# ShawnNew/Detectron2-CenterNet

Measured on AMD Instinct MI355X. Metric: images/sec at 512x512 (infer bs=64), higher is better.
Workload: dtype f16x3

## Files before the change

### detectron2-centernet_amd/csrc/api.hip

```cpp
#include "conv_common.h"
#include "../../include/ctdet_hip.h"
#include <stdarg.h>
#include <stdio.h>
#include <string.h>
#include <stdlib.h>
#include <atomic>

static thread_local char g_err[512] = "";
void ctdet_set_error(const char* fmt, ...) {
  va_list ap;
  va_start(ap, fmt);
  vsnprintf(g_err, sizeof(g_err), fmt, ap);
  va_end(ap);
}

thread_local int g_label_mode = 0;
static thread_local char g_label[128] = "";
bool ctdet_set_label(const char* fmt, ...) {
  va_list ap;
  va_start(ap, fmt);
  vsnprintf(g_label, sizeof(g_label), fmt, ap);
  va_end(ap);
  return g_label_mode == 2;
}
// ... 12 lines not shown
size_t dwconv3x3_wgrad_workspace_bytes(int, int, int, int, int);
int launch_dwconv3x3(const void*, int, const float*, void*, int, int, int, int, int, int, int, int, hipStream_t);
int launch_dwconv3x3_wgrad(const void*, int, const void*, int, float*, float*, float, int, int, int, int, int, int, hipStream_t);
size_t decode_workspace_bytes(int B, int H, int W, int C, int K);
int decode_status_words(int H, int W, int C, int K, long* ws_words, int* below_word);
int launch_decode(const DecArgs&, hipStream_t);
int launch_postprocess(const float*, const float*, const int*, int, int, int, float, const float*, float*, float*, int*,
                       int*, hipStream_t);
int launch_gaussian_radius(const int*, int, double*, int*, hipStream_t);
int launch_gaussian_targets(const float*, const int64_t*, const int*, int, int, int, int, int, float*, float*, float*,
                            int64_t*, uint8_t*, hipStream_t);
size_t focal_workspace_bytes(long numel);
int launch_focal_loss(const float*, const float*, const float*, int, int, int, int, float, void*, float*, float*, float*,
                      hipStream_t);
int launch_reg_l1(const float*, int, const uint8_t*, const int64_t*, const float*, int, int, int, float, float*, float*,
                  int, hipStream_t);
int launch_sgd(float*, const float*, float*, long, const float*, float, float, int, hipStream_t);
int launch_sgd_runs(float*, const float*, float*, long, const long*, const int*, const float*, const float*, int, float, int,
                    hipStream_t);

struct WgradArgs {
  const void* x; const void* dy; float* dw;
  int B, H, W, Cin, in_stride, Cout, Ho, Wo, dy_stride, R, S, stride, pad, dil, K, M, msplit;
  float scale;
  int lw, lh;
  int perm_rs, perm_cin, cin_real, cout_real;
};
int launch_grad_scatter_oihw(const void* const*, void* const*, const int*, const int*, const int*, const int*, int, hipStream_t);
int launch_pack_weights_batch(const void*, int, int, hipStream_t);
int launch_pack_weights_x3(const float*, void*, float*, int, int, int, int, int, int, int, int, int, int, hipStream_t);
int launch_pack_weights_x3_batch(const void*, int, int, hipStream_t);
int launch_split_weights(const float*, void*, long, hipStream_t);
bool dcn_offset_fused_ok(const ConvArgs& a);
int conv_pair_korder(const ConvArgs& a);
bool head_fused_x_ok(const HeadArgs& a, bool x3);
bool dcn_split_window_ok(const ConvArgs& a);
size_t chan_reduce_workspace_bytes(int C);
int launch_bn_train_fwd(const f16*, int, const f16*, int, f16*, int, int, int, const float*, const float*, float, float,
                        float*, float*, float*, float*, float*, float*, void*, int, hipStream_t);
int launch_bn_train_bwd(const f16*, int, const f16*, int, const f16*, int, const float*, const float*, const float*, int,
                        int, int, f16*, int, f16*, int, float*, float*, float, void*, hipStream_t);
int launch_conv_wgrad(const WgradArgs&, hipStream_t);
int launch_conv_wgrad_f32(const WgradArgs&, hipStream_t);
int launch_conv_wgrad_x3(const WgradArgs&, hipStream_t);
int launch_bn_train_fwd_f32(const float*, int, const float*, int, float*, int, int, int, const float*, const float*, float,
                            float, float*, float*, float*, float*, float*, float*, void*, int, hipStream_t);
int launch_bn_train_bwd_f32(const float*, int, const float*, int, const float*, int, const float*, const float*, const float*,
                            int, int, int, float*, int, float*, int, float*, float*, float, void*, hipStream_t);
int launch_bn_local_stats(const void*, int, int, int, int, int, double*, void*, int, hipStream_t);
int launch_bn_sync_fwd(const void*, int, const void*, int, void*, int, int, int, const double*, int, const float*, const float*,
                       float, float, float*, float*, float*, float*, float*, float*, int, int, hipStream_t);
int launch_bn_local_grad_sums(const void*, int, const void*, int, const void*, int, const float*, const float*, int, int, int, int,
                              int, double*, float*, float*, float, void*, int, hipStream_t);
int launch_bn_sync_bwd(const void*, int, const void*, int, const void*, int, const float*, const float*, const float*,
                       const double*, const double*, int, int, int, int, void*, int, void*, int, int, hipStream_t);
int launch_maxpool2x2_bwd_f32(const float*, int, const float*, int, float*, int, int, int, int, int, hipStream_t);
int launch_maxpool3x3s2_bwd(const void*, int, const void*, int, void*, int, int, int, int, int, int, int, int, int, hipStream_t);
int launch_ese_dot(const void*, int, const void*, int, int, int, int, int, float*, hipStream_t);
int launch_ese_bwd(const void*, int, const float*, const float*, void*, int, int, int, int, int, hipStream_t);
int launch_dwconvT_bwd_f32(const float*, int, const float*, int, const float*, float*, int, float*, int, int, int, int, int,
                           hipStream_t);
int launch_dcn_cols_f32(const float*, int, const float*, int, float*, int, int, int, int, int, hipStream_t);
int launch_dcn_col2im_coord_f32(const float*, const float*, int, const float*, int, float*, float*, int, int, int, int, int, int,
                                int, int, hipStream_t);
int launch_dcn_col2im_fused(const float*, int, int, const void*, const float*, const float*, int, const float*, int, float*, float*, int,
                            int, int, int, int, int, hipStream_t);
// ... 141 lines not shown
  }
  CTDET_CHECK(false, "dcnv2: bad compute dtype %d", d->compute_dtype);
}

int32_t ctdet_dcnv2_cols_supported(const ctdet_conv_desc* d, const void* x, const void* y) {
  ConvArgs a;
  if (fill_args(d, a) || d->compute_dtype != CTDET_DT_F16X3 || d->out_dtype != CTDET_DT_F32) return 0;
  a.x = x; a.y = const_cast<void*>(y);
  return dcn_split_window_ok(a) ? 1 : 0;
}

int32_t ctdet_dcnv2_fwd_cols(const ctdet_conv_desc* d, const void* x, const float* offset_mask, int32_t om_stride,
                             int32_t mask_is_prob, const void* w_packed, const float* scale, const float* bias, void* y,
                             float* cols_out, void* stream) {
  ConvArgs a;
  int rc = fill_args(d, a);
  if (rc) return rc;
  if (a.M == 0) return 0;
  CTDET_CHECK(x && w_packed && y && offset_mask && cols_out, "dcnv2_fwd_cols: null pointer");
  CTDET_CHECK(mask_is_prob >= CTDET_DCN_MASK_LOGIT && mask_is_prob <= CTDET_DCN_MASK_NONE, "dcnv2: mask mode %d", mask_is_prob);
  CTDET_CHECK(om_stride >= (mask_is_prob == CTDET_DCN_MASK_NONE ? 2 : 3) * d->R * d->S, "dcnv2: om_stride=%d < %d*R*S", om_stride,
              mask_is_prob == CTDET_DCN_MASK_NONE ? 2 : 3);
  CTDET_CHECK(d->compute_dtype == CTDET_DT_F16X3 && d->out_dtype == CTDET_DT_F32 && (((size_t)cols_out) & 15) == 0,
              "dcnv2_fwd_cols: the f16x3 mode's entry point (f32 tensors), 16-byte aligned columns");
  a.x = x; a.w = w_packed; a.scale = scale; a.bias = bias; a.res = nullptr; a.y = y;
  a.om = offset_mask; a.om_stride = om_stride; a.mask_is_prob = mask_is_prob;
  CTDET_CHECK(dcn_split_window_ok(a), "dcnv2_fwd_cols: shape not served by the LDS-window kernel (ask ctdet_dcnv2_cols_supported first)");
  a.cols_out = cols_out;
  return launch_conv_f32(a, true, true, (hipStream_t)stream);
}

int32_t ctdet_dcnv2_offset_supported(const ctdet_conv_desc* d) {
  ConvArgs a;
  if (fill_args(d, a) || d->compute_dtype != CTDET_DT_F16) return 0;
  a.y = nullptr;
  return dcn_offset_fused_ok(a) ? 1 : 0;
}

int32_t ctdet_dcnv2_offset_fwd(const ctdet_conv_desc* d, const void* x, const void* w_off_packed, const float* b_off,
                               float* om_out, int32_t om_out_stride, const void* w_packed, const float* scale,
                               const float* bias, void* y, void* stream) {
  ConvArgs a;
  int rc = fill_args(d, a);
  if (rc) return rc;
  if (a.M == 0) return 0;
  CTDET_CHECK(x && w_off_packed && b_off && w_packed && y, "dcnv2_offset: null pointer");
  CTDET_CHECK(d->compute_dtype == CTDET_DT_F16, "dcnv2_offset: f16 only");
  CTDET_CHECK(!om_out || (om_out_stride >= 28 && om_out_stride % 4 == 0 && ((size_t)om_out & 15) == 0),
              "dcnv2_offset: om_out needs a 16-byte aligned row of >= 28 floats (stride %d)", om_out_stride);
  a.x = x; a.w = w_packed; a.scale = scale; a.bias = bias; a.res = nullptr; a.y = y;
  a.w_off = w_off_packed; a.b_off = b_off; a.om_out = om_out; a.om_out_stride = om_out_stride;
  return launch_conv_f16(a, d->out_dtype, true, (hipStream_t)stream);
}

int32_t ctdet_preprocess(const void* img, int32_t img_dtype, void* out, int32_t out_dtype, int32_t B, int32_t H,
                         int32_t W, int32_t Hp, int32_t Wp, int64_t img_batch_stride, const float* mean3,
                         const float* std3, int32_t out_stride, int32_t border, void* stream) {
  CTDET_CHECK(img && out && mean3 && std3, "preprocess: null pointer");
  return launch_preprocess(img, img_dtype, out, out_dtype, B, H, W, Hp, Wp, (long)img_batch_stride, mean3, std3,
                           out_stride, border, (hipStream_t)stream);
}

static int head_args(const ctdet_head_desc* d, HeadArgs& a) {
  a.nheads = d->nheads; a.B = d->B; a.H = d->H; a.W = d->W; a.Cin = d->Cin; a.in_stride = d->in_stride;
  a.clamp_lo = d->clamp_lo; a.clamp_hi = d->clamp_hi;
  CTDET_CHECK(d->nheads >= 1 && d->nheads <= 4, "head_fused: nheads=%d out of range", d->nheads);
  for (int h = 0; h < d->nheads; ++h) {
    CTDET_CHECK(d->w2[h] && d->b2[h] && d->y[h], "head_fused: head %d: null pointer", h);
    a.w2[h] = d->w2[h]; a.b2[h] = (const float*)d->b2[h]; a.y[h] = (float*)d->y[h];
    a.y_stride[h] = d->y_stride[h]; a.cout[h] = d->cout[h]; a.act[h] = d->act[h];
  }
  return 0;
}

int32_t ctdet_head_fused_supported(int32_t compute_dtype, int32_t H, int32_t W, int32_t Cin, int32_t in_stride, const void* x) {
  HeadArgs a = {};
  a.x = x; a.H = H; a.W = W; a.Cin = Cin; a.in_stride = in_stride;
  if (compute_dtype != CTDET_DT_F16 && compute_dtype != CTDET_DT_F16X3) return 0;
  return head_fused_x_ok(a, compute_dtype == CTDET_DT_F16X3) ? 1 : 0;
}
// ... 457 lines not shown
```

### detectron2-centernet_amd/csrc/conv_f32.hip

```cpp
#include "conv_common.h"

template <int BP, int BC, int WP, int WC_, bool SP>
__global__ void __launch_bounds__(256) conv_f32_mfma_kernel(const ConvArgs a) {
  constexpr int KS = 16, EPV = 4;
  constexpr int TP = BP / WP / 16;
  constexpr int TC = BC / WC_ / 16;
  constexpr int A_LD = BP / 64;
  constexpr int BCL = BC < 64 ? 64 : BC;
  constexpr int B_LD = BCL / 64;
  constexpr int NLOAD = A_LD + B_LD;
  constexpr int STAGE = (BP + BCL) * 64;
  constexpr int NST = 3;
  static_assert(WP * WC_ == 4, "4 waves per workgroup");
  __shared__ __attribute__((aligned(16))) char smem[NST * STAGE];

  const int tid = threadIdx.x, lane = tid & 63;
  const int wave = __builtin_amdgcn_readfirstlane(tid >> 6);
  const int wp = wave / WC_, wc = wave % WC_;
  int m_tile, n_tile;
  if (!tile_of_block((a.M + BP - 1) / BP, a.Cout_pad / BC, m_tile, n_tile)) return;
  const int m0 = m_tile * BP, n0 = n_tile * BC;
  const float* __restrict__ x = (const float*)a.x;
  const float* __restrict__ w = (const float*)a.w;
  const float* zero = (const float*)g_zero_page;
// ... 626 lines not shown
    if (T == 8 && chunk + 1 < nch) {
      wait_vmcnt<0>();
      __builtin_amdgcn_s_barrier();
      asm volatile("" ::: "memory");
      sample(0, chunk + 1, pfn);
    }
#pragma unroll
    for (int p = 0; p < TP; ++p) pf[p] = pfn[p];
    if (TS < 2) {
#pragma unroll
      for (int c = 0; c < TC; ++c) wf[c] = wfn[c];
    }
  };
  for (int chunk = 0; chunk < nch; ++chunk) {
    const int s = chunk * 3;
    tap(s, chunk, std::integral_constant<int, 0>{});
    tap(s, chunk, std::integral_constant<int, 1>{});
    tap(s, chunk, std::integral_constant<int, 2>{});
    tap(s + 1, chunk, std::integral_constant<int, 3>{});
    tap(s + 1, chunk, std::integral_constant<int, 4>{});
    tap(s + 1, chunk, std::integral_constant<int, 5>{});
    tap(s + 2, chunk, std::integral_constant<int, 6>{});
    tap(s + 2, chunk, std::integral_constant<int, 7>{});
    tap(s + 2, chunk, std::integral_constant<int, 8>{});
  }

#pragma unroll
  for (int p = 0; p < TP; ++p) {
    const int m = (b * a.H + ty0 + prow) * a.W + tx0 + 8 * p + pcol;
    epilogue_tiles<float, TC>(a, m, n0, q, acc[p]);
  }
}

template <int TP, int BC, bool COLS = false, bool NM = false>
__global__ void __launch_bounds__(512 / TP, (TP == 1 && BC == 64) ? 4 : 2) dcn_split_window_kernel(const ConvArgs a) {
  constexpr int TH = 8, TW = 16, BP = 128, MG = 4;
  constexpr int NT = 512 / TP;
  static_assert(BC * 4 <= NT, "at most one weight piece per thread and tap (waves beyond BC / 16 fetch none)");
  constexpr int WR = TH + 2 + 2 * MG, WCOLS = TW + 2 + 2 * MG;
  constexpr int NPIECE = WR * WCOLS * 4;
  constexpr int W_LD = (NPIECE + NT - 1) / NT;
  constexpr int WINB = ((NPIECE + 63) / 64) * 1024;
  constexpr int GEOW = 9 * BP * 16, GEOC = 9 * BP * 4;
  constexpr int TC = BC / 16;
  constexpr int WST = BC * 64, NST = 2, STG = 3 * WST;
  static_assert(WINB + GEOW + GEOC + NST * STG <= ((TP == 2 || BC == 64) ? 81920 : 163840), "two workgroups / one (128 couts) per CU");
  __shared__ __attribute__((aligned(16))) char smem[WINB + GEOW + GEOC + NST * STG];
  char* const win = smem;
  char* const geow = smem + WINB;
  char* const geoc = smem + WINB + GEOW;
  char* const ring = smem + WINB + GEOW + GEOC;

  const int tid = threadIdx.x, lane = tid & 63;
  const int wave = __builtin_amdgcn_readfirstlane(tid >> 6);
  const int tiles_x = a.W / TW, tiles_y = a.H / TH;
  int m_tile, n_tile;
  if (!tile_of_block(a.B * tiles_y * tiles_x, a.Cout_pad / BC, m_tile, n_tile)) return;
  const int tx0 = (m_tile % tiles_x) * TW;
  const int ty0 = ((m_tile / tiles_x) % tiles_y) * TH;
  const int b = m_tile / (tiles_x * tiles_y);
  const int n0 = n_tile * BC;
  const float* zero = (const float*)g_zero_page;
  asm volatile("" : "+v"(zero));
  const float* ximg = (const float*)a.x + (long)b * a.H * a.W * a.in_stride;
  const int wy0 = ty0 - 1 - MG, wx0 = tx0 - 1 - MG;
  const int nch = a.Cin / 16;

  const int lrow = tid >> 2, slotw = tid & 3;
  const int gwk = slotw ^ swz(lrow);
  const float* wptr;
  {
    const int tt = lrow >> 4, r = lrow & 15;
    wptr = (const float*)a.w + (long)(n0 + cout_of<TC>(tt, r >> 2, r & 3)) * a.Kpad + gwk * 4;
  }
  auto issue_w = [&](int chunk, int tr, int st) {
    if (BC * 4 < NT && wave >= BC / 16) return;
#pragma unroll
    for (int ts = 0; ts < 3; ++ts)
      dma16(wptr + (tr * 3 + ts) * a.Cin + chunk * 16, ring + st * STG + ts * WST + wave * 1024);
  };
  int wofs[W_LD];
#pragma unroll
  for (int i = 0; i < W_LD; ++i) {
    const int pid = tid + NT * i;
    const int pw = pid >> 2, sl = pid & 3;
    const int wr = pw / WCOLS, wcn = pw - wr * WCOLS;
    const int y = wy0 + wr, x = wx0 + wcn;
    const bool ok = pid < NPIECE && y >= 0 && y < a.H && x >= 0 && x < a.W;
    wofs[i] = ok ? (y * a.W + x) * a.in_stride + (sl ^ (2 * (wr & 1))) * 4 : -1;
  }
  auto issue_window = [&](int chunk) {
#pragma unroll
    for (int i = 0; i < W_LD; ++i) {
      if (i < W_LD - 1 || (wave * 64 + NT * i) * 16 < WINB) {
        int o = wofs[i];
        asm volatile("" : "+v"(o));
        dma16(o >= 0 ? ximg + o + chunk * 16 : zero, win + (wave * 64 + NT * i) * 16);
      }
    }
  };
  issue_window(0);
  issue_w(0, 0, 0);

  {
    constexpr int GS = NT / 128;
    const int gp = tid & 127, gh = tid >> 7;
    const int py = ty0 + (gp >> 4), pxx = tx0 + (gp & 15);
    const float* omrow = a.om + ((long)(b * a.H + py) * a.W + pxx) * a.om_stride;
#pragma unroll
    for (int i = 0; i < (9 + GS - 1) / GS; ++i) {
      const int t = GS * i + gh;
      if (t < 9) {
        const int tr = t / 3, ts = t - 3 * tr;
        const float h_im = (float)(py - 1 + tr) + omrow[2 * t], w_im = (float)(pxx - 1 + ts) + omrow[2 * t + 1];
        const float mraw = NM ? 1.f : omrow[18 + t];
        const bool valid = h_im > -1.f && w_im > -1.f && h_im < (float)a.H && w_im < (float)a.W;
        const float mk = valid ? ((NM || a.mask_is_prob) ? mraw : ctdet_sigmoid_exact(mraw)) : 0.f;
        const float fh = floorf(h_im), fw = floorf(w_im);
        const int h_low = (int)fh, w_low = (int)fw;
        const float lh = valid ? h_im - fh : 0.f, lw = valid ? w_im - fw : 0.f, hh = 1.f - lh, hw = 1.f - lw;
        const int wr = h_low - wy0, wcn = w_low - wx0;
        const bool inside = wr >= 0 && wr + 1 < WR && wcn >= 0 && wcn + 1 < WCOLS;
        const bool oow = valid && !inside;
        const unsigned code = (valid && inside) ? ((unsigned)((wr * WCOLS + wcn) * 64) | ((unsigned)(wr & 1) << 5)) : (oow ? 0x80000000u : 0u);
        f32x4 gv;
        gv[0] = hh * hw * mk; gv[1] = hh * lw * mk; gv[2] = lh * hw * mk; gv[3] = lh * lw * mk;
        *(f32x4*)(geow + (t * BP + gp) * 16) = gv;
        *(unsigned*)(geoc + (t * BP + gp) * 4) = code;
      }
    }
  }
  wait_vmcnt<0>();
  __syncthreads();
  const int fr = lane & 15, q = lane >> 4;
  const int prow = TP == 2 ? 2 * wave + (fr >> 3) : wave, pcol = TP == 2 ? (fr & 7) : fr;
  const unsigned q4 = (unsigned)q << 4;

  struct Raw { f32x4 w[TP], v[TP][4]; };
  auto gather = [&](int t, int chunk, Raw& r) {
    unsigned code[TP];
    unsigned far = 0;
#pragma unroll
    for (int p = 0; p < TP; ++p) {
      const int px = prow * 16 + (TP == 2 ? 8 * p : 0) + pcol;
      r.w[p] = *(const f32x4*)(geow + (t * BP + px) * 16);
      code[p] = *(const unsigned*)(geoc + (t * BP + px) * 4);
      far |= code[p] >> 31;
    }
    const bool any_far = __builtin_amdgcn_ballot_w64(far != 0) != 0;
#pragma unroll
    for (int p = 0; p < TP; ++p) {
      const unsigned A = (code[p] & 0xFFFFu) ^ q4;
      const char* c0p = win + A;
      const char* c2p = win + (A ^ 32u) + WCOLS * 64;
      r.v[p][0] = *(const f32x4*)(c0p); r.v[p][1] = *(const f32x4*)(c0p + 64);
      r.v[p][2] = *(const f32x4*)(c2p); r.v[p][3] = *(const f32x4*)(c2p + 64);
      if (any_far) {
        const bool out = code[p] >> 31;
        const int py = ty0 + prow, pxx = tx0 + (TP == 2 ? 8 * p : 0) + pcol, tr = t / 3, ts = t - 3 * (t / 3);
        const float* omrow = a.om + ((long)(b * a.H + py) * a.W + pxx) * a.om_stride;
        float dh, dw;
        gload2_sync(omrow + 2 * t, dh, dw);
        const float h_im = (float)(py - 1 + tr) + dh, w_im = (float)(pxx - 1 + ts) + dw;
        const int h_low = (int)floorf(h_im), w_low = (int)floorf(w_im);
        const bool r0 = out && h_low >= 0, r1 = out && h_low + 1 <= a.H - 1, c0 = w_low >= 0, c1 = w_low + 1 <= a.W - 1;
        const long o0 = ((long)h_low * a.W + w_low) * a.in_stride, o2 = o0 + (long)a.W * a.in_stride;
        const float* base = ximg + chunk * 16 + q * 4;
        if (out) {
          gload4_sync_into((r0 && c0) ? base + o0 : zero, r.v[p][0]);
          gload4_sync_into((r0 && c1) ? base + o0 + a.in_stride : zero, r.v[p][1]);
          gload4_sync_into((r1 && c0) ? base + o2 : zero, r.v[p][2]);
          gload4_sync_into((r1 && c1) ? base + o2 + a.in_stride : zero, r.v[p][3]);
        }
      }
    }
  };
  float* const colp = (COLS && n0 == 0) ? a.cols_out + q * 4 : nullptr;
  auto blend = [&](const Raw& r, f16x8 (&b1)[TP], f16x8 (&b2)[TP], int t, int chunk) {
#pragma unroll
    for (int p = 0; p < TP; ++p) {
      f32x4 val;
#pragma unroll
      for (int e = 0; e < 4; ++e)
        val[e] = r.w[p][0] * r.v[p][0][e] + r.w[p][1] * r.v[p][1][e] + r.w[p][2] * r.v[p][2][e] + r.w[p][3] * r.v[p][3][e];
      if constexpr (COLS) {
        if (colp) {
          const long m = (long)(b * a.H + ty0 + prow) * a.W + tx0 + (TP == 2 ? 8 * p : 0) + pcol;
          *(f32x4*)(colp + m * (9L * a.Cin) + t * a.Cin + chunk * 16) = val;
        }
      }
      split_b(val, b1[p], b2[p]);
    }
  };

  f32x4 acc[TP][TC];
#pragma unroll
  for (int p = 0; p < TP; ++p)
// ... 399 lines not shown
    if (vec && !deform) {
      const int rc = launch_halo_split(a, s);
      if (rc <= 0) return rc;
    }
  }
  if (deform)
    return a.mask_is_prob == DCN_MASK_NONE ? launch_f32_deform<SP, true>(a, vec, bc, s) : launch_f32_deform<SP, false>(a, vec, bc, s);
  if (vec) {
    const bool big = ((long)a.M + 255) / 256 * (a.Cout_pad / bc) >= 512;
    const int kind = f32_uniform_k_ok(a) ? 1 : 0;
    switch (bc) {
      case 16: return launch_f32_mfma<256, 16, 4, 1, SP>(a, kind, s);
      case 32: return big ? launch_f32_mfma<256, 32, 4, 1, SP>(a, kind, s) : launch_f32_mfma<128, 32, 4, 1, SP>(a, kind, s);
      case 64: return big ? launch_f32_mfma<256, 64, 4, 1, SP>(a, kind, s) : launch_f32_mfma<128, 64, 2, 2, SP>(a, kind, s);
      case 128: return big ? launch_f32_mfma<256, 128, 2, 2, SP>(a, kind, s) : launch_f32_mfma<128, 128, 2, 2, SP>(a, kind, s);
    }
  }
  const int CP = (a.Cout + 3) & ~3;
  const long total = (long)a.M * CP;
  dim3 grid((unsigned)((total + 255) / 256));
  CTDET_KERNEL("conv_direct_%s_kernel<conv>", sp_name<SP>());
  hipLaunchKernelGGL((conv_direct_f32_kernel<false, SP>), grid, dim3(256), 0, s, a);
  CTDET_LAUNCH_CHECK();
  return 0;
}

bool dcn_split_window_ok(const ConvArgs& a) {
  const int bc = pick_bc(a.Cout);
  return f32_vector_ok(a, bc) && a.Cin % 16 == 0 && a.nsrc <= 1 && a.R == 3 && a.S == 3 && a.stride == 1 && a.pad == 1 && a.dil == 1 &&
         a.H % 8 == 0 && a.W % 16 == 0 && a.H <= 4094 && a.W <= 4094 && a.Kpad == a.K && a.Cout_pad % 64 == 0 && a.korder == 0 &&
         !(ctdet_tuning_flags() & (CTDET_TUNE_NO_F32_DCN_WINDOW | CTDET_TUNE_DCN_WINDOW_V1));
}

int launch_conv_f32(const ConvArgs& a, bool deform, bool split, hipStream_t s) {
  return split ? launch_conv_f32_t<true>(a, deform, s) : launch_conv_f32_t<false>(a, deform, s);
}

__global__ void __launch_bounds__(256) split_weights_kernel(const f32x4* __restrict__ src, f16x8* __restrict__ dst, long groups) {
  const long i = (long)blockIdx.x * 256 + threadIdx.x;
  if (i >= groups) return;
  const f32x4 w = src[i];
  f16x8 o;
#pragma unroll
  for (int j = 0; j < 4; ++j) {
    const f16 h = (f16)w[j];
    o[j] = h;
    o[4 + j] = (f16)(w[j] - (float)h);
  }
  dst[i] = o;
}

int launch_split_weights(const float* src, void* dst, long n, hipStream_t s) {
  CTDET_CHECK(n % 4 == 0 && (((size_t)src | (size_t)dst) & 15) == 0, "split_weights: needs 16-byte aligned buffers of a multiple of 4 floats");
  if (n == 0) return 0;
  const long groups = n / 4;
  hipLaunchKernelGGL(split_weights_kernel, dim3((unsigned)((groups + 255) / 256)), dim3(256), 0, s, (const f32x4*)src, (f16x8*)dst,
                     groups);
  CTDET_LAUNCH_CHECK();
  return 0;
}
```

### detectron2-centernet_amd/layers/deform_conv.py

```python
import math

import torch
from torch import nn
from torch.nn.modules.utils import _pair

from .. import ops
from ..ops import ACT_NONE, ACT_RELU, DCN_MASK_NONE, DCN_MASK_PROB, F16, F32
from . import hipnn


def _check_supported(groups, deformable_groups, stride, dilation):
    if groups != 1 or deformable_groups != 1:
        raise NotImplementedError("HIP DCNv2 supports groups=1, deformable_groups=1 (all CenterNet uses)")


def modulated_deform_conv(input, offset, mask, weight, bias=None, stride=1, padding=0, dilation=1, groups=1,
                          deformable_groups=1):
    if not input.is_cuda:
        raise NotImplementedError("Deformable Conv is not supported on CPUs!")
    _check_supported(groups, deformable_groups, stride, dilation)
    return _deform_conv_nchw(input, [offset, mask], weight, bias, stride, padding, dilation, DCN_MASK_PROB,
                             "modulated_deform_conv")


# ... 85 lines not shown
                                  self.groups, self.deformable_groups)
        if self.norm is not None:
            x = self.norm(x)
        if self.activation is not None:
            x = self.activation(x)
        return x


class DCN(nn.Module):

    def __init__(self, in_channels, out_channels, kernel_size, stride, padding, dilation=1, deformable_groups=1):
        super().__init__()
        _check_supported(1, deformable_groups, stride, dilation)
        self.in_channels, self.out_channels = in_channels, out_channels
        self.kernel_size = _pair(kernel_size)
        self.stride, self.padding, self.dilation = stride, padding, dilation
        self.deformable_groups = deformable_groups
        self.weight = nn.Parameter(torch.Tensor(out_channels, in_channels, *self.kernel_size))
        self.bias = nn.Parameter(torch.Tensor(out_channels))
        n = in_channels * self.kernel_size[0] * self.kernel_size[1]
        stdv = 1.0 / math.sqrt(n)
        self.weight.data.uniform_(-stdv, stdv)
        self.bias.data.zero_()
        kh, kw = self.kernel_size
        self.conv_offset_mask = nn.Conv2d(in_channels, deformable_groups * 3 * kh * kw, kernel_size=self.kernel_size,
                                          stride=stride, padding=padding, bias=True)
        self.conv_offset_mask.weight.data.zero_()
        self.conv_offset_mask.bias.data.zero_()

    def hip_forward(self, x, ctx, bn=None, act=ACT_NONE):
        p = hipnn.packed(self, "dcn", ctx.compute, self.weight, bn, self.bias, self.stride, self.padding, self.dilation,
                         cout_align=64 if ctx.compute == F16 else None)
        com = self.conv_offset_mask
        if ctx.compute == F16 and x.shape[3] % 32 == 0:
            p_off = hipnn.packed(com, "conv", ctx.compute, com.weight, None, com.bias, com.stride[0], com.padding[0], com.dilation[0])
            if ops.dcnv2_offset_supported(x, p_off, p):
                return ops.dcnv2_offset(x, p_off, p, act=act)
        om = hipnn.conv_module(x, com, None, ACT_NONE, ctx=ctx, out_dtype=torch.float32)
        return ops.dcnv2(x, om, p, act=act)

    def forward(self, x):
        ctx = hipnn.Ctx(F16 if x.dtype == torch.float16 else F32)
        xh = x.permute(0, 2, 3, 1).contiguous()
        if torch.is_grad_enabled() and (x.requires_grad or self.weight.requires_grad):
            from ..ops_train import ConvFn, DCNFn
            om = ConvFn.apply(xh, self.conv_offset_mask.weight, self.conv_offset_mask.bias, self.stride, self.padding,
                              False, True, 1.0)
            y = DCNFn.apply(xh, om, self.weight, self.bias, False, 1.0)
        else:
            y = self.hip_forward(xh, ctx)
        return hipnn.to_nchw_view(y, self.out_channels)


class DeformConvV2(nn.Module):

    def __init__(self, chi, cho):
        super().__init__()
        self.actf = nn.Sequential(nn.BatchNorm2d(cho, momentum=0.1), nn.ReLU(inplace=True))
        self.conv = DCN(chi, cho, kernel_size=(3, 3), stride=1, padding=1, dilation=1, deformable_groups=1)
        nn.init.uniform_(self.actf[0].weight.data)

    def hip_forward(self, x, ctx):
        return self.conv.hip_forward(x, ctx, bn=self.actf[0], act=ACT_RELU)

    def forward(self, x):
        ctx = hipnn.Ctx(F16 if x.dtype == torch.float16 else F32)
        return hipnn.to_nchw_view(self.hip_forward(hipnn.to_nhwc(x, ctx), ctx), self.conv.out_channels)
# ... 1 lines not shown
```

### detectron2-centernet_amd/ops.py

```python
import ctypes as C
import os
import math

import torch

from . import _lib
from ._lib import (ACT_NONE, ACT_RELU, ACT_SIGMOID_CLAMP, DCN_MASK_LOGIT, DCN_MASK_NONE, DCN_MASK_PROB, F16, F16X3, F32, U8,
                   ConvDesc, HeadDesc)

_TORCH_DT = {F16: torch.float16, F32: torch.float32}

PROFILE_ON = False
PROFILE = []
PROFILE_REP = 5


class _Prof:
    def __init__(self, p, M, deform, out_dt, nsrc=1, flops=None):
        self.on = PROFILE_ON
        if self.on:
            _lib.lib().ctdet_set_label_mode(1)
            self.flops = flops if flops is not None else 2.0 * M * p.Cout * p.R * p.S * p.Cin_real
            osz = 2 if out_dt == F16 else 4
            if p is not None:
# ... 494 lines not shown
    mask_is_prob = int(mask_is_prob)
    if mask_is_prob not in (DCN_MASK_LOGIT, DCN_MASK_PROB, DCN_MASK_NONE):
        raise ValueError(f"dcnv2: mask mode {mask_is_prob}")
    if p.compute == F16 and p.Cout_pad % 64:
        raise ValueError(f"dcnv2 (f16) works on 64-cout tiles: pack the weights with PackedConv(..., cout_align=64) "
                         f"(Cout={p.Cout}, packed rows {p.Cout_pad})")
    if out is None and p.compute == F16 and p.Cout_eff % 8:
        B, H, W, _ = x.shape
        dt = out_dtype if out_dtype is not None else torch.float16
        out = torch.empty(B, H, W, round_up(p.Cout_eff, 8), dtype=dt, device=x.device)[..., :p.Cout_eff]
    out = _alloc_out(x, p, out, out_dtype)
    assert tuple(offset_mask.shape[:3]) == tuple(out.shape[:3])
    p._wp_scaled = None
    d = p.desc(x, out, act, None)
    cols = None
    if want_cols and p.compute == F16X3 and _lib.lib().ctdet_dcnv2_cols_supported(C.byref(d), _ptr(x), _ptr(out)):
        cols = torch.empty(x.shape[0], x.shape[1], x.shape[2], 9 * p.Cin, dtype=torch.float32, device=x.device)
    prof = _Prof(p, d.B * d.Ho * d.Wo, True, d.out_dtype)
    if prof.on and cols is not None:
        prof.bytes += cols.numel() * 4
    for _ in range(prof.reps()):
        if cols is not None:
            rc = _lib.lib().ctdet_dcnv2_fwd_cols(C.byref(d), _ptr(x), _ptr(offset_mask), _nhwc_stride(offset_mask), int(mask_is_prob),
                                                 _ptr(p.w), _ptr(p.scale), _ptr(p.bias), _ptr(out), _ptr(cols), _stream())
        else:
            rc = _lib.lib().ctdet_dcnv2_fwd(C.byref(d), _ptr(x), _ptr(offset_mask), _nhwc_stride(offset_mask),
                                            int(mask_is_prob), _ptr(p.w), _ptr(p.scale), _ptr(p.bias), _ptr(out), _stream())
    _lib.check(rc, "ctdet_dcnv2_fwd")
    prof.done()
    _range_check(out, p, "dcnv2")
    return (out, cols) if want_cols else out


def dcnv2_offset_supported(x, p_off, p):
    if p.compute != F16 or p_off.compute != F16 or p.Cout_pad != 64 or p_off.Cout != 27 or p_off.Cout_pad != 32:
        return False
    if (p_off.R, p_off.S, p_off.stride, p_off.pad, p_off.dil, p_off.korder, p_off.Kpad) != (3, 3, 1, 1, 1, 1, p.Kpad):
        return False
    B, H, W, _ = x.shape
    out = torch.empty(0, H, W, round_up(p.Cout_eff, 8), dtype=torch.float16, device=x.device)
    d = p.desc(x[:0], out, ACT_NONE, None)
    d.B = B
    return bool(_lib.lib().ctdet_dcnv2_offset_supported(C.byref(d)))


def dcnv2_offset(x, p_off, p, out=None, act=ACT_NONE, out_dtype=None, om_out=None):
    _require_cuda(x, out, om_out)
    assert dt_of(x) == F16 and p.compute == F16 and p_off.bias is not None and p_off.scale is None
    if out is None and p.Cout_eff % 8:
        B, H, W, _ = x.shape
        dt = out_dtype if out_dtype is not None else torch.float16
        out = torch.empty(B, H, W, round_up(p.Cout_eff, 8), dtype=dt, device=x.device)[..., :p.Cout_eff]
    out = _alloc_out(x, p, out, out_dtype)
    assert p_off.bias.shape[0] >= 28
    d = p.desc(x, out, act, None)
    prof = _Prof(p, d.B * d.Ho * d.Wo, True, d.out_dtype, flops=2.0 * d.B * d.Ho * d.Wo * p.K * (p.Cout + 27))
    if prof.on:
        prof.bytes -= d.B * d.Ho * d.Wo * 27 * 4
    for _ in range(prof.reps()):
        rc = _lib.lib().ctdet_dcnv2_offset_fwd(C.byref(d), _ptr(x), _ptr(p_off.w), _ptr(p_off.bias), _ptr(om_out),
                                               _nhwc_stride(om_out) if om_out is not None else 0, _ptr(p.w), _ptr(p.scale),
                                               _ptr(p.bias), _ptr(out), _stream())
    _lib.check(rc, "ctdet_dcnv2_offset_fwd")
    prof.done()
    return out


def preprocess(images, mean, std, Hp, Wp, out_dtype=torch.float16, out=None, partial=False, border=0):
    _require_cuda(images)
    B, Cc, H, W = images.shape
    assert Cc == 3 and images.stride(3) == 1 and images.stride(2) == W and images.stride(1) == H * W
    if out is None:
        if border:
            out = torch.zeros(B, Hp + 2 * border, Wp + 2 * border, 8, dtype=out_dtype, device=images.device)
        else:
            out = torch.empty(B, Hp, Wp, 8, dtype=out_dtype, device=images.device)
    assert out.shape[3] % 8 == 0 or (out.shape[3] == 4 and out.dtype == torch.float32)
    assert tuple(out.shape[1:3]) == (Hp + 2 * border, Wp + 2 * border)
    m = (C.c_float * 3)(*[float(v) for v in mean])
    s = (C.c_float * 3)(*[float(v) for v in std])
    rc = _lib.lib().ctdet_preprocess(_ptr(images), dt_of(images), _ptr(out), dt_of(out), B, H, W, Hp, Wp,
                                     images.stride(0), m, s, _nhwc_stride(out), int(border), _stream())
    _lib.check(rc, "ctdet_preprocess")
    return out


class PackedDlaBase:

    def __init__(self, w_stem, sb_stem, w_l0, sb_l0, w_l1, sb_l1):
        assert tuple(w_stem.shape) == (16, 3, 7, 7) and tuple(w_l0.shape) == (16, 16, 3, 3) and tuple(w_l1.shape) == (32, 16, 3, 3)
        dev = w_stem.device
        w4 = torch.zeros(16, 7, 8, 4, dtype=torch.float32, device=dev)
        w4[:, :, :7, :3] = w_stem.detach().float().permute(0, 2, 3, 1)
        self.w0 = w4.reshape(16, 224).to(torch.float16).contiguous()
        self.p1 = PackedConv(w_l0, sb_l0[0], sb_l0[1], stride=1, pad=1, compute=F16)
        self.p2 = PackedConv(w_l1, sb_l1[0], sb_l1[1], stride=2, pad=1, compute=F16)
        assert self.p1.korder == 0 and self.p1.Kpad == 160 and self.p2.korder == 0 and self.p2.Kpad == 160
# ... 415 lines not shown
```

Measured before the change: 4000.

## Fuse offset/mask conv into the f16x3 DCNv2 window kernel for inference

Adds an f16x3 path that computes the 3x3 offset/mask convolution inside the DCNv2 split-window kernel. Each tile loads a halo of the f32 input, splits it into hi/lo f16 parts in LDS, and runs MFMA over the offset weights. The offset tile is kept in LDS and read directly when building the bilinear sampling tables, and far-sample coordinates are packed into the code word. This removes the separate offset conv launch and the global write and reread of the offset/mask tensor, at the cost of a more complex LDS schedule and extra work per DCN tile.

```diff
diff --git a/detectron2-centernet_amd/csrc/api.hip b/detectron2-centernet_amd/csrc/api.hip
--- a/detectron2-centernet_amd/csrc/api.hip
+++ b/detectron2-centernet_amd/csrc/api.hip
@@ -68,6 +68,8 @@
 int launch_pack_weights_x3_batch(const void*, int, int, hipStream_t);
 int launch_split_weights(const float*, void*, long, hipStream_t);
 bool dcn_offset_fused_ok(const ConvArgs& a);
+bool dcn_offset_fused_x3_ok(const ConvArgs& a);
+int launch_dcn_offset_x3(const ConvArgs& a, hipStream_t s);
 int conv_pair_korder(const ConvArgs& a);
 bool head_fused_x_ok(const HeadArgs& a, bool x3);
 bool dcn_split_window_ok(const ConvArgs& a);
@@ -275,8 +277,10 @@
 
 int32_t ctdet_dcnv2_offset_supported(const ctdet_conv_desc* d) {
   ConvArgs a;
-  if (fill_args(d, a) || d->compute_dtype != CTDET_DT_F16) return 0;
+  if (fill_args(d, a)) return 0;
   a.y = nullptr;
+  if (d->compute_dtype == CTDET_DT_F16X3) return (d->out_dtype == CTDET_DT_F32 && dcn_offset_fused_x3_ok(a)) ? 1 : 0;
+  if (d->compute_dtype != CTDET_DT_F16) return 0;
   return dcn_offset_fused_ok(a) ? 1 : 0;
 }
 
@@ -288,7 +292,13 @@
   if (rc) return rc;
   if (a.M == 0) return 0;
   CTDET_CHECK(x && w_off_packed && b_off && w_packed && y, "dcnv2_offset: null pointer");
-  CTDET_CHECK(d->compute_dtype == CTDET_DT_F16, "dcnv2_offset: f16 only");
+  if (d->compute_dtype == CTDET_DT_F16X3) {
+    CTDET_CHECK(d->out_dtype == CTDET_DT_F32 && !om_out, "dcnv2_offset(f16x3): f32 output, no om_out (inference form)");
+    a.x = x; a.w = w_packed; a.scale = scale; a.bias = bias; a.res = nullptr; a.y = y;
+    a.w_off = w_off_packed; a.b_off = b_off; a.mask_is_prob = DCN_MASK_LOGIT;
+    return launch_dcn_offset_x3(a, (hipStream_t)stream);
+  }
+  CTDET_CHECK(d->compute_dtype == CTDET_DT_F16, "dcnv2_offset: f16 or f16x3");
   CTDET_CHECK(!om_out || (om_out_stride >= 28 && om_out_stride % 4 == 0 && ((size_t)om_out & 15) == 0),
               "dcnv2_offset: om_out needs a 16-byte aligned row of >= 28 floats (stride %d)", om_out_stride);
   a.x = x; a.w = w_packed; a.scale = scale; a.bias = bias; a.res = nullptr; a.y = y;
diff --git a/detectron2-centernet_amd/csrc/conv_f32.hip b/detectron2-centernet_amd/csrc/conv_f32.hip
--- a/detectron2-centernet_amd/csrc/conv_f32.hip
+++ b/detectron2-centernet_amd/csrc/conv_f32.hip
@@ -682,8 +682,9 @@
   }
 }
 
-template <int TP, int BC, bool COLS = false, bool NM = false>
+template <int TP, int BC, bool COLS = false, bool NM = false, bool FUS = false>
 __global__ void __launch_bounds__(512 / TP, (TP == 1 && BC == 64) ? 4 : 2) dcn_split_window_kernel(const ConvArgs a) {
+  static_assert(!FUS || (TP == 2 && BC == 64 && !COLS && !NM), "the fused offset conv: inference form of the 64-cout DCNv2 tile");
   constexpr int TH = 8, TW = 16, BP = 128, MG = 4;
   constexpr int NT = 512 / TP;
   static_assert(BC * 4 <= NT, "at most one weight piece per thread and tap (waves beyond BC / 16 fetch none)");
@@ -749,21 +750,204 @@
       }
     }
   };
-  issue_window(0);
-  issue_w(0, 0, 0);
+  constexpr int OMS = 33;
+  float* const om_lds = (float*)geow;
+  if constexpr (FUS) {
+    constexpr int HPC = (TH + 2) * (TW + 2) * 4;
+    constexpr int H_LD = (HPC + NT - 1) / NT;
+    constexpr int HB = H_LD * NT * 16;
+    constexpr int WSTEP = 2 * 32 * 64;
+    static_assert(NT == 256 && 2 * HB <= WINB && 9 * WSTEP <= GEOW + GEOC + NST * STG, "LDS layout of the offset conv");
+    static_assert(BP * OMS * 4 <= GEOW, "the offset tile lives in the weight table's space");
+    static_assert(sizeof(smem) <= 81920, "two workgroups per CU");
+    char* const halo = win;
+    char* const wimg = geow;
+    int hofs[H_LD];
+#pragma unroll
+    for (int i = 0; i < H_LD; ++i) {
+      const int j = tid + NT * i;
+      const int hp = j >> 2, sl = j & 3;
+      const int hr = hp / (TW + 2), hc = hp - hr * (TW + 2);
+      const int y = ty0 - 1 + hr, x = tx0 - 1 + hc;
+      const bool ok = j < HPC && y >= 0 && y < a.H && x >= 0 && x < a.W;
+      hofs[i] = ok ? (y * a.W + x) * a.in_stride + (sl ^ swz(hc)) * 4 : -1;
+    }
+    auto issue_halo = [&](int chunk, int hb) {
+#pragma unroll
+      for (int i = 0; i < H_LD; ++i) {
+        int o = hofs[i];
+        asm volatile("" : "+v"(o));
+        dma16(o >= 0 ? ximg + o + chunk * 16 : zero, halo + hb * HB + (wave * 64 + NT * i) * 16);
+      }
+    };
+    auto convert = [&](int hb) {
+      char* base = halo + hb * HB + tid * 16;
+      f32x4 v[H_LD];
+#pragma unroll
+      for (int i = 0; i < H_LD; ++i) v[i] = *(const f32x4*)(base + i * NT * 16);
+#pragma unroll
+      for (int i = 0; i < H_LD; ++i) {
+        const f16x4 hi = __builtin_convertvector(v[i], f16x4);
+        f32x4 r;
+#pragma unroll
+        for (int e = 0; e < 4; ++e) r[e] = v[i][e] - (float)hi[e];
+        const f16x4 lo = __builtin_convertvector(r, f16x4);
+        *(f16x8*)(base + i * NT * 16) = __builtin_shufflevector(hi, lo, 0, 1, 2, 3, 4, 5, 6, 7);
+      }
+    };
+    const int orow = a.Cin / 32 * 288;
+    const float* wsrc;
+    {
+      const int img = tid >> 7, lr = (tid >> 2) & 31, sl = tid & 3;
+      wsrc = (const float*)a.w_off + (long)cout_of<2>(lr >> 4, (lr & 15) >> 2, lr & 3) * orow + img * 16 + (sl ^ swz(lr)) * 4;
+    }
+    auto issue_wseg = [&](int pair, int s0, int s1) {
+      for (int s_ = s0; s_ < s1; ++s_) dma16(wsrc + (pair * 9 + s_) * 32, wimg + s_ * WSTEP + wave * 1024);
+    };
+    const int l15 = lane & 15, kg = lane >> 4;
+    int pb[3];
+#pragma unroll
+    for (int S_ = 0; S_ < 3; ++S_) pb[S_] = (l15 + S_) * 64 + ((kg ^ swz(l15 + S_)) << 4);
+    const char* wfrag = wimg + l15 * 64 + ((kg ^ swz(l15)) << 4);
+    const bool w32 = a.W % 32 == 0;
+    const bool ordb[2] = {w32 ? false : (wave & 1) != 0, w32 ? true : (wave & 1) != 0};
+    typedef unsigned long long u64;
+    typedef u64 u64x2 __attribute__((ext_vector_type(2)));
+    typedef __attribute__((address_space(3))) const volatile u64 lds_u64;
+    f32x4 oacc[2][2];
+#pragma unroll
+    for (int u = 0; u < 2; ++u)
+#pragma unroll
+      for (int c = 0; c < 2; ++c) oacc[u][c] = (f32x4){0.f, 0.f, 0.f, 0.f};
+    auto step = [&](auto sc) {
+      constexpr int S = decltype(sc)::value;
+      constexpr int B0 = S <= 4 ? 0 : 1, B1 = S < 4 ? 0 : 1;
+      constexpr int T0 = S < 4 ? 2 * S : (S == 4 ? 8 : 2 * (S - 5)), T1 = S < 4 ? 2 * S + 1 : (S == 4 ? 8 : 2 * (S - 5) + 1);
+      f16x8 xw[2], yw[2];
+#pragma unroll
+      for (int c = 0; c < 2; ++c) {
+        xw[c] = *(const f16x8*)(wfrag + S * WSTEP + c * 1024);
+        yw[c] = *(const f16x8*)(wfrag + S * WSTEP + 2048 + c * 1024);
+      }
+      u64x2 hq[2], lq[2];
+#pragma unroll
+      for (int u = 0; u < 2; ++u) {
+        const char* s0 = halo + B0 * HB + (2 * wave + u + T0 / 3) * ((TW + 2) * 64) + pb[T0 % 3];
+        const char* s1 = halo + B1 * HB + (2 * wave + u + T1 / 3) * ((TW + 2) * 64) + pb[T1 % 3];
+        hq[u][0] = *(lds_u64*)s0; hq[u][1] = *(lds_u64*)s1;
+        lq[u][0] = *(lds_u64*)(s0 + 8); lq[u][1] = *(lds_u64*)(s1 + 8);
+      }
+#pragma unroll
+      for (int u = 0; u < 2; ++u) {
+        const f16x8 H = __builtin_bit_cast(f16x8, hq[u]), L = __builtin_bit_cast(f16x8, lq[u]);
+        if (ordb[u]) {
+#pragma unroll
+          for (int c = 0; c < 2; ++c) oacc[u][c] = __builtin_amdgcn_mfma_f32_16x16x32_f16(xw[c], L, oacc[u][c], 0, 0, 0);
+#pragma unroll
+          for (int c = 0; c < 2; ++c) oacc[u][c] = __builtin_amdgcn_mfma_f32_16x16x32_f16(xw[c], H, oacc[u][c], 0, 0, 0);
+#pragma unroll
+          for (int c = 0; c < 2; ++c) oacc[u][c] = __builtin_amdgcn_mfma_f32_16x16x32_f16(yw[c], H, oacc[u][c], 0, 0, 0);
+        } else {
+#pragma unroll
+          for (int c = 0; c < 2; ++c) oacc[u][c] = __builtin_amdgcn_mfma_f32_16x16x32_f16(xw[c], H, oacc[u][c], 0, 0, 0);
+#pragma unroll
+          for (int c = 0; c < 2; ++c) oacc[u][c] = __builtin_amdgcn_mfma_f32_16x16x32_f16(yw[c], H, oacc[u][c], 0, 0, 0);
+#pragma unroll
+          for (int c = 0; c < 2; ++c) oacc[u][c] = __builtin_amdgcn_mfma_f32_16x16x32_f16(xw[c], L, oacc[u][c], 0, 0, 0);
+        }
+      }
+    };
+    const int npair = a.Cin / 32;
+    issue_halo(0, 0);
+    issue_halo(1, 1);
+    issue_wseg(0, 0, 9);
+    wait_vmcnt<0>();
+    convert(0);
+    convert(1);
+    __syncthreads();
+    for (int pair = 0; pair < npair; ++pair) {
+      const bool last = pair + 1 == npair;
+      step(std::integral_constant<int, 0>{});
+      step(std::integral_constant<int, 1>{});
+      step(std::integral_constant<int, 2>{});
+      step(std::integral_constant<int, 3>{});
+      if (pair > 0) {
+        wait_vmcnt<0>();
+        convert(1);
+      }
+      __syncthreads();
+      step(std::integral_constant<int, 4>{});
+      __syncthreads();
+      if (!last) {
+        issue_halo(2 * pair + 2, 0);
+        issue_wseg(pair + 1, 0, 5);
+      }
+      step(std::integral_constant<int, 5>{});
+      step(std::integral_constant<int, 6>{});
+      step(std::integral_constant<int, 7>{});
+      step(std::integral_constant<int, 8>{});
+      if (!last) {
+        wait_vmcnt<0>();
+        convert(0);
+      }
+      __syncthreads();
+      if (!last) {
+        issue_halo(2 * pair + 3, 1);
+        issue_wseg(pair + 1, 5, 9);
+      }
+    }
+#pragma unroll
+    for (int u = 0; u < 2; ++u)
+#pragma unroll
+      for (int c = 0; c < 2; ++c) {
+        const int c0 = cout_of<2>(c, kg, 0);
+        f32x4 v = oacc[u][c];
+        const f32x4 sv = *(const f32x4*)(a.b_off + 32 + c0);
+        v = v * sv;
+        const f32x4 bv = *(const f32x4*)(a.b_off + c0);
+        v = v + bv;
+        asm volatile("" : "+v"(v));
+        oacc[u][c] = v;
+      }
+    issue_window(0);
+    issue_w(0, 0, 0);
+#pragma unroll
+    for (int u = 0; u < 2; ++u)
+#pragma unroll
+      for (int c = 0; c < 2; ++c) {
+        float* dst = om_lds + ((2 * wave + u) * 16 + l15) * OMS + cout_of<2>(c, kg, 0);
+#pragma unroll
+        for (int e = 0; e < 4; ++e) dst[e] = oacc[u][c][e];
+      }
+    __syncthreads();
+  } else {
+    issue_window(0);
+    issue_w(0, 0, 0);
+  }
 
   {
     constexpr int GS = NT / 128;
+    constexpr int GN = (9 + GS - 1) / GS;
     const int gp = tid & 127, gh = tid >> 7;
     const int py = ty0 + (gp >> 4), pxx = tx0 + (gp & 15);
-    const float* omrow = a.om + ((long)(b * a.H + py) * a.W + pxx) * a.om_stride;
-#pragma unroll
-    for (int i = 0; i < (9 + GS - 1) / GS; ++i) {
+    const float* omrow = FUS ? om_lds + gp * OMS : a.om + ((long)(b * a.H + py) * a.W + pxx) * a.om_stride;
+    float fdh[FUS ? GN : 1], fdw[FUS ? GN : 1], fmk[FUS ? GN : 1];
+    if constexpr (FUS) {
+#pragma unroll
+      for (int i = 0; i < GN; ++i) {
+        const int t = GS * i + gh;
+        if (t < 9) { fdh[i] = omrow[2 * t]; fdw[i] = omrow[2 * t + 1]; fmk[i] = omrow[18 + t]; }
+      }
+      __syncthreads();
+    }
+#pragma unroll
+    for (int i = 0; i < GN; ++i) {
       const int t = GS * i + gh;
       if (t < 9) {
         const int tr = t / 3, ts = t - 3 * tr;
-        const float h_im = (float)(py - 1 + tr) + omrow[2 * t], w_im = (float)(pxx - 1 + ts) + omrow[2 * t + 1];
-        const float mraw = NM ? 1.f : omrow[18 + t];
+        const float odh = FUS ? fdh[FUS ? i : 0] : omrow[2 * t], odw = FUS ? fdw[FUS ? i : 0] : omrow[2 * t + 1];
+        const float h_im = (float)(py - 1 + tr) + odh, w_im = (float)(pxx - 1 + ts) + odw;
+        const float mraw = NM ? 1.f : (FUS ? fmk[FUS ? i : 0] : omrow[18 + t]);
         const bool valid = h_im > -1.f && w_im > -1.f && h_im < (float)a.H && w_im < (float)a.W;
         const float mk = valid ? ((NM || a.mask_is_prob) ? mraw : ctdet_sigmoid_exact(mraw)) : 0.f;
         const float fh = floorf(h_im), fw = floorf(w_im);
@@ -772,7 +956,8 @@
         const int wr = h_low - wy0, wcn = w_low - wx0;
         const bool inside = wr >= 0 && wr + 1 < WR && wcn >= 0 && wcn + 1 < WCOLS;
         const bool oow = valid && !inside;
-        const unsigned code = (valid && inside) ? ((unsigned)((wr * WCOLS + wcn) * 64) | ((unsigned)(wr & 1) << 5)) : (oow ? 0x80000000u : 0u);
+        const unsigned farcode = FUS ? (0x80000000u | ((unsigned)(h_low + 1) << 16) | ((unsigned)(w_low + 1) << 4)) : 0x80000000u;
+        const unsigned code = (valid && inside) ? ((unsigned)((wr * WCOLS + wcn) * 64) | ((unsigned)(wr & 1) << 5)) : (oow ? farcode : 0u);
         f32x4 gv;
         gv[0] = hh * hw * mk; gv[1] = hh * lw * mk; gv[2] = lh * hw * mk; gv[3] = lh * lw * mk;
         *(f32x4*)(geow + (t * BP + gp) * 16) = gv;
@@ -808,11 +993,16 @@
       if (any_far) {
         const bool out = code[p] >> 31;
         const int py = ty0 + prow, pxx = tx0 + (TP == 2 ? 8 * p : 0) + pcol, tr = t / 3, ts = t - 3 * (t / 3);
-        const float* omrow = a.om + ((long)(b * a.H + py) * a.W + pxx) * a.om_stride;
-        float dh, dw;
-        gload2_sync(omrow + 2 * t, dh, dw);
-        const float h_im = (float)(py - 1 + tr) + dh, w_im = (float)(pxx - 1 + ts) + dw;
-        const int h_low = (int)floorf(h_im), w_low = (int)floorf(w_im);
+        int h_low, w_low;
+        if constexpr (FUS) {
+          h_low = (int)((code[p] >> 16) & 0xFFFu) - 1; w_low = (int)((code[p] >> 4) & 0xFFFu) - 1;
+        } else {
+          const float* omrow = a.om + ((long)(b * a.H + py) * a.W + pxx) * a.om_stride;
+          float dh, dw;
+          gload2_sync(omrow + 2 * t, dh, dw);
+          const float h_im = (float)(py - 1 + tr) + dh, w_im = (float)(pxx - 1 + ts) + dw;
+          h_low = (int)floorf(h_im); w_low = (int)floorf(w_im);
+        }
         const bool r0 = out && h_low >= 0, r1 = out && h_low + 1 <= a.H - 1, c0 = w_low >= 0, c1 = w_low + 1 <= a.W - 1;
         const long o0 = ((long)h_low * a.W + w_low) * a.in_stride, o2 = o0 + (long)a.W * a.in_stride;
         const float* base = ximg + chunk * 16 + q * 4;
@@ -1278,6 +1468,24 @@
          !(ctdet_tuning_flags() & (CTDET_TUNE_NO_F32_DCN_WINDOW | CTDET_TUNE_DCN_WINDOW_V1));
 }
 
+bool dcn_offset_fused_x3_ok(const ConvArgs& a) {
+  return dcn_split_window_ok(a) && a.Cin % 32 == 0 && a.Cout_pad == 64 && !a.res && !(ctdet_tuning_flags() & CTDET_TUNE_DCN_SPLIT_8W64);
+}
+
+int launch_dcn_offset_x3(const ConvArgs& a, hipStream_t s) {
+  CTDET_CHECK((long)a.B * a.H * a.W * a.in_stride < (1L << 31), "dcnv2_offset(f16x3): input too large for 32-bit element offsets");
+  CTDET_CHECK(dcn_offset_fused_x3_ok(a) && aligned16(a.w_off) && aligned16(a.b_off) && !a.cols_out && !a.om_out &&
+                  a.mask_is_prob == DCN_MASK_LOGIT,
+              "dcnv2_offset(f16x3): needs 3x3/s1/p1, Cin %% 32 == 0, a map divisible by 8x16, 64 packed couts and 16-byte aligned "
+              "operands (Cin=%d, %dx%d, Cout_pad=%d; ctdet_dcnv2_offset_supported)", a.Cin, a.H, a.W, a.Cout_pad);
+  const int nbx = a.B * (a.H / 8) * (a.W / 16);
+  dim3 grid(8 * ((nbx + 7) / 8));
+  CTDET_KERNEL("dcn_f16x3_window_kernel<8x16,64,offset conv fused>");
+  hipLaunchKernelGGL((dcn_split_window_kernel<2, 64, false, false, true>), grid, dim3(256), 0, s, a);
+  CTDET_LAUNCH_CHECK();
+  return 0;
+}
+
 int launch_conv_f32(const ConvArgs& a, bool deform, bool split, hipStream_t s) {
   return split ? launch_conv_f32_t<true>(a, deform, s) : launch_conv_f32_t<false>(a, deform, s);
 }
diff --git a/detectron2-centernet_amd/layers/deform_conv.py b/detectron2-centernet_amd/layers/deform_conv.py
--- a/detectron2-centernet_amd/layers/deform_conv.py
+++ b/detectron2-centernet_amd/layers/deform_conv.py
@@ -141,7 +141,8 @@
         p = hipnn.packed(self, "dcn", ctx.compute, self.weight, bn, self.bias, self.stride, self.padding, self.dilation,
                          cout_align=64 if ctx.compute == F16 else None)
         com = self.conv_offset_mask
-        if ctx.compute == F16 and x.shape[3] % 32 == 0:
+        fused_x3 = ctx.compute == ops.F16X3 and ops.DCN_X3_FUSED and not ops.RANGE_CHECK
+        if (ctx.compute == F16 or fused_x3) and x.shape[3] % 32 == 0:
             p_off = hipnn.packed(com, "conv", ctx.compute, com.weight, None, com.bias, com.stride[0], com.padding[0], com.dilation[0])
             if ops.dcnv2_offset_supported(x, p_off, p):
                 return ops.dcnv2_offset(x, p_off, p, act=act)
diff --git a/detectron2-centernet_amd/ops.py b/detectron2-centernet_amd/ops.py
--- a/detectron2-centernet_amd/ops.py
+++ b/detectron2-centernet_amd/ops.py
@@ -550,13 +550,42 @@
     return (out, cols) if want_cols else out
 
 
+DCN_X3_FUSED = os.environ.get("CTDET_NO_FUSED_DCN_X3", "0") != "1"
+
+
+def _off_operands_x3(p_off):
+    if p_off.w_pair is None or p_off.pair_korder != 3:
+        if p_off._x3_src is not None and p_off._pair_capable and p_off.Cin % 32 == 0:
+            p_off.pair_korder = 3
+            p_off.w_pair, p_off.scale_pair = p_off._x3_operand(3)
+        elif p_off._wp_scaled is not None and p_off.w_pair is None and p_off.Cin % 32 == 0:
+            (p_off.w_pair, p_off.pair_korder), p_off._wp_scaled = p_off._pack_pairs(p_off._wp_scaled), None
+        else:
+            return None
+    sc = p_off.scale_pair if p_off.scale_pair is not None else p_off.scale
+    hit = p_off.__dict__.get("_off_bs")
+    if hit is None or hit[0] is not sc or hit[1] is not p_off.bias:
+        bs = torch.zeros(64, dtype=torch.float32, device=p_off.w_pair.device)
+        bs[:p_off.bias.shape[0]] = p_off.bias
+        bs[32:32 + sc.shape[0]] = sc
+        hit = p_off._off_bs = (sc, p_off.bias, bs)
+    return p_off.w_pair, hit[2]
+
+
 def dcnv2_offset_supported(x, p_off, p):
-    if p.compute != F16 or p_off.compute != F16 or p.Cout_pad != 64 or p_off.Cout != 27 or p_off.Cout_pad != 32:
+    if p.compute not in (F16, F16X3) or p_off.compute != p.compute or p.Cout_pad != 64 or p_off.Cout != 27:
         return False
-    if (p_off.R, p_off.S, p_off.stride, p_off.pad, p_off.dil, p_off.korder, p_off.Kpad) != (3, 3, 1, 1, 1, 1, p.Kpad):
+    if (p_off.R, p_off.S, p_off.stride, p_off.pad, p_off.dil) != (3, 3, 1, 1, 1) or p_off.bias is None:
         return False
     B, H, W, _ = x.shape
-    out = torch.empty(0, H, W, round_up(p.Cout_eff, 8), dtype=torch.float16, device=x.device)
+    if p.compute == F16X3:
+        if dt_of(x) != F32 or x.data_ptr() % 16 or p.Cin % 32 or p_off.Cin != p.Cin or _off_operands_x3(p_off) is None:
+            return False
+        out = torch.empty(0, H, W, p.Cout_eff, dtype=torch.float32, device=x.device)
+    else:
+        if p_off.Cout_pad != 32 or (p_off.korder, p_off.Kpad) != (1, p.Kpad):
+            return False
+        out = torch.empty(0, H, W, round_up(p.Cout_eff, 8), dtype=torch.float16, device=x.device)
     d = p.desc(x[:0], out, ACT_NONE, None)
     d.B = B
     return bool(_lib.lib().ctdet_dcnv2_offset_supported(C.byref(d)))
@@ -564,8 +593,18 @@
 
 def dcnv2_offset(x, p_off, p, out=None, act=ACT_NONE, out_dtype=None, om_out=None):
     _require_cuda(x, out, om_out)
-    assert dt_of(x) == F16 and p.compute == F16 and p_off.bias is not None and p_off.scale is None
-    if out is None and p.Cout_eff % 8:
+    assert dt_of(x) == p.act_dt and p.compute in (F16, F16X3) and p_off.compute == p.compute and p_off.bias is not None
+    if p.compute == F16X3:
+        assert om_out is None, "dcnv2_offset (f16x3) keeps no offsets: the inference form"
+        ops_off = _off_operands_x3(p_off)
+        if ops_off is None:
+            raise ValueError("dcnv2_offset (f16x3): the offset conv has no korder-3 pair image (3x3/s1/p1, Cin % 32 == 0)")
+        w_off, b_off = ops_off
+        p._wp_scaled = None
+    else:
+        assert p_off.scale is None
+        w_off, b_off = p_off.w, p_off.bias
+    if out is None and p.compute == F16 and p.Cout_eff % 8:
         B, H, W, _ = x.shape
         dt = out_dtype if out_dtype is not None else torch.float16
         out = torch.empty(B, H, W, round_up(p.Cout_eff, 8), dtype=dt, device=x.device)[..., :p.Cout_eff]
@@ -576,11 +615,13 @@
     if prof.on:
         prof.bytes -= d.B * d.Ho * d.Wo * 27 * 4
     for _ in range(prof.reps()):
-        rc = _lib.lib().ctdet_dcnv2_offset_fwd(C.byref(d), _ptr(x), _ptr(p_off.w), _ptr(p_off.bias), _ptr(om_out),
+        rc = _lib.lib().ctdet_dcnv2_offset_fwd(C.byref(d), _ptr(x), _ptr(w_off), _ptr(b_off), _ptr(om_out),
                                                _nhwc_stride(om_out) if om_out is not None else 0, _ptr(p.w), _ptr(p.scale),
                                                _ptr(p.bias), _ptr(out), _stream())
     _lib.check(rc, "ctdet_dcnv2_offset_fwd")
     prof.done()
+    if p.compute == F16X3:
+        _range_check(out, p, "dcnv2_offset")
     return out
 
 
```

New measurement: 4082 (median of 6 runs). +2.1%, better.
